# lisvulaczo/lodestar

Measured on AMD Instinct MI355X. Metric: BLS signature sets verified/sec (whole node) at 1/2/4/8 MI355X; p50 batch latency, higher is better.
Workload: dtype u32

## Files before the change

### lodestar_amd/csrc/lsg_curve.hpp

```cpp
#pragma once
#include "lsg_tower.hpp"

LSG_INL fp_t fadd(const fp_t& a, const fp_t& b) { return fp_add(a, b); }
LSG_INL fp2_t fadd(const fp2_t& a, const fp2_t& b) { return fp2_add(a, b); }
LSG_INL fp_t fsub(const fp_t& a, const fp_t& b) { return fp_sub(a, b); }
LSG_INL fp2_t fsub(const fp2_t& a, const fp2_t& b) { return fp2_sub(a, b); }
LSG_INL fp_t fmul(const fp_t& a, const fp_t& b) { return fp_mul(a, b); }
LSG_INL fp2_t fmul(const fp2_t& a, const fp2_t& b) { return fp2_mul(a, b); }
LSG_INL fp_t fsqr(const fp_t& a) { return fp_sqr(a); }
LSG_INL fp2_t fsqr(const fp2_t& a) { return fp2_sqr(a); }
LSG_INL fp_t fneg(const fp_t& a) { return fp_neg(a); }
LSG_INL fp2_t fneg(const fp2_t& a) { return fp2_neg(a); }
LSG_INL fps_t<1, 0> fsum(const fp_t& a) { return fps(a); }
LSG_INL fp2s_t<1, 0> fsum(const fp2_t& a) { return fp2s(a); }
template <int K, int P, int N>
LSG_INL fps_t<K * P, K * N> fsum_mulk(const fps_t<P, N>& a) { return fps_mulk<K>(a); }
template <int K, int P0, int N0, int P1, int N1>
LSG_INL fp2s_t<K * P0, K * N0, K * P1, K * N1> fsum_mulk(const fp2s_t<P0, N0, P1, N1>& a) { return fp2s_mulk<K>(a); }
template <int K> LSG_INL fp_t fmulk(const fp_t& a) { return fp_mulk<K>(a); }
template <int K> LSG_INL fp2_t fmulk(const fp2_t& a) { return fp2_mulk<K>(a); }
template <class F> LSG_INL F fsub2(const F& a, const F& b, const F& c) { return (fsum(a) - b - c).carry(); }
LSG_INL fp_t fmul_b3(const fp_t& a) { return fp_mul12(a); }
LSG_INL fp2_t fmul_b3(const fp2_t& a) { return fp2_mul_b3(a); }
template <int P0, int N0, int P1, int N1>
// ... 47 lines not shown

template <class F>
LSG_INL proj_t<F> proj_from_aff(const aff_t<F>& a) {
  proj_t<F> r;
  r.X = a.x;
  r.Y = a.y;
  r.Z = fone<F>();
  return r;
}

template <class F>
LSG_INL bool proj_is_inf(const proj_t<F>& a) {
  return fis_zero(a.Z);
}

template <class F>
LSG_INL proj_t<F> proj_neg(const proj_t<F>& a) {
  proj_t<F> r = a;
  r.Y = fneg(a.Y);
  return r;
}

template <class F>
LSG_INL proj_t<F> proj_add(const proj_t<F>& p, const proj_t<F>& q) {
  F t0 = fmul(p.X, q.X);
  F t1 = fmul(p.Y, q.Y);
  F t2 = fmul(p.Z, q.Z);
  F t3 = fsub2(fmul(fadd(p.X, p.Y), fadd(q.X, q.Y)), t0, t1);
  F t4 = fsub2(fmul(fadd(p.Y, p.Z), fadd(q.Y, q.Z)), t1, t2);
  F Y3 = fsub2(fmul(fadd(p.X, p.Z), fadd(q.X, q.Z)), t0, t2);
  F X3;
  t0 = fmulk<3>(t0);
  t2 = fmul_b3(t2);
  F Z3 = fadd(t1, t2);
  t1 = fsub(t1, t2);
  Y3 = fmul_b3(Y3);
  X3 = fmul(t4, Y3);
  t2 = fmul(t3, t1);
  X3 = fsub(t2, X3);
  Y3 = fmul(Y3, t0);
  t1 = fmul(t1, Z3);
  Y3 = fadd(t1, Y3);
  t0 = fmul(t0, t3);
  Z3 = fmul(Z3, t4);
  Z3 = fadd(Z3, t0);
  proj_t<F> r;
  r.X = X3;
  r.Y = Y3;
  r.Z = Z3;
  return r;
}

template <class F>
LSG_INL proj_t<F> proj_add_mixed(const proj_t<F>& p, const aff_t<F>& q) {
  F t0 = fmul(p.X, q.x);
  F t1 = fmul(p.Y, q.y);
  F t3 = fsub2(fmul(fadd(q.x, q.y), fadd(p.X, p.Y)), t0, t1);
  F t4 = fadd(fmul(q.y, p.Z), p.Y);
  F Y3 = fadd(fmul(q.x, p.Z), p.X);
  F X3;
  t0 = fmulk<3>(t0);
  F t2 = fmul_b3(p.Z);
  F Z3 = fadd(t1, t2);
  t1 = fsub(t1, t2);
  Y3 = fmul_b3(Y3);
  X3 = fmul(t4, Y3);
  t2 = fmul(t3, t1);
  X3 = fsub(t2, X3);
  Y3 = fmul(Y3, t0);
  t1 = fmul(t1, Z3);
  Y3 = fadd(t1, Y3);
  t0 = fmul(t0, t3);
  Z3 = fmul(Z3, t4);
  Z3 = fadd(Z3, t0);
  proj_t<F> r;
  r.X = X3;
  r.Y = Y3;
  r.Z = Z3;
  return r;
}

template <class F>
LSG_INL proj_t<F> proj_dbl(const proj_t<F>& p) {
  F t0 = fsqr(p.Y);
  F Z3 = fmulk<8>(t0);
  F t1 = fmul(p.Y, p.Z);
  F t2 = fmul_b3(fsqr(p.Z));
  F X3 = fmul(t2, Z3);
  F Y3 = fadd(t0, t2);
  Z3 = fmul(t1, Z3);
  t0 = fsub(t0, fmulk<3>(t2));
  Y3 = fmul(t0, Y3);
  Y3 = fadd(X3, Y3);
  t1 = fmul(p.X, p.Y);
  X3 = fmulk<2>(fmul(t0, t1));
  proj_t<F> r;
  r.X = X3;
  r.Y = Y3;
  r.Z = Z3;
  return r;
}

LSG_BIGFN g1p_t g1_add(g1p_t p, g1p_t q) { return proj_add(p, q); }
LSG_BIGFN g1p_t g1_add_mixed(g1p_t p, g1a_t q) { return proj_add_mixed(p, q); }
LSG_BIGFN g1p_t g1_dbl(g1p_t p) { return proj_dbl(p); }
LSG_BIGFN g2p_t g2_add(g2p_t p, g2p_t q) { return proj_add(p, q); }
LSG_BIGFN g2p_t g2_dbl(g2p_t p) { return proj_dbl(p); }
LSG_BIGFN g2p_t g2_add_mixed(g2p_t p, g2a_t q) { return proj_add_mixed(p, q); }

LSG_INL g1p_t gadd(const g1p_t& p, const g1p_t& q) { return g1_add(p, q); }
LSG_INL g2p_t gadd(const g2p_t& p, const g2p_t& q) { return g2_add(p, q); }
LSG_INL g1p_t gdbl(const g1p_t& p) { return g1_dbl(p); }
LSG_INL g2p_t gdbl(const g2p_t& p) { return g2_dbl(p); }
#ifdef LSG_FP2_LANES
typedef aff_t<fp2v_t> g2va_t;
typedef proj_t<fp2v_t> g2vp_t;
LSG_BIGFN g2vp_t g2v_add(g2vp_t p, g2vp_t q) { return proj_add(p, q); }
LSG_INL g2vp_t gadd(const g2vp_t& p, const g2vp_t& q) { return g2v_add(p, q); }
LSG_INL g2va_t g2v_from_pair(const g2a_t& a) { return g2va_t{fp2v_from_pair(a.x), fp2v_from_pair(a.y)}; }
LSG_INL g2vp_t g2v_from_pair(const g2p_t& p) {
  return g2vp_t{fp2v_from_pair(p.X), fp2v_from_pair(p.Y), fp2v_from_pair(p.Z)};
}
LSG_INL g2p_t g2_to_pair(const g2vp_t& p) {
  g2p_t r;
  r.X = fp2v_to_pair(p.X);
  r.Y = fp2v_to_pair(p.Y);
  r.Z = fp2v_to_pair(p.Z);
  return r;
}
#endif
LSG_INL const g2p_t& g2_to_pair(const g2p_t& p) { return p; }
template <class F> struct g2_layout;
template <> struct g2_layout<fp2_t> {
  static LSG_INL g2a_t in(const g2a_t& a) { return a; }
};
#ifdef LSG_FP2_LANES
template <> struct g2_layout<fp2v_t> {
  static LSG_INL g2va_t in(const g2a_t& a) { return g2v_from_pair(a); }
};
typedef fp2v_t chain_fp2_t;
#else
typedef fp2_t chain_fp2_t;
#endif

template <class F>
struct jac_t {
  F X, Y, Z;
};

template <class F>
LSG_INL jac_t<F> jac_from_proj(const proj_t<F>& p) {
  F zz = fsqr(p.Z);
  jac_t<F> r;
  bool inf = fis_zero(p.Z);
  r.X = fselect(inf, fone<F>(), fmul(p.X, p.Z));
  r.Y = fselect(inf, fone<F>(), fmul(p.Y, zz));
  r.Z = p.Z;
  return r;
}

template <class F>
LSG_INL proj_t<F> jac_to_proj(const jac_t<F>& p) {
  F zz = fsqr(p.Z);
  proj_t<F> r;
  bool inf = fis_zero(p.Z);
  r.X = fmul(p.X, p.Z);
  r.Y = fselect(inf, fone<F>(), p.Y);
  r.Z = fmul(zz, p.Z);
  return r;
}

template <class F>
LSG_INL jac_t<F> jac_dbl_t(const jac_t<F>& p) {
  F A = fsqr(p.X);
  F B = fsqr(p.Y);
  F C = fsqr(B);
  F D = (fsum(fsqr(fadd(p.X, B))) - A - C).template carry_mul<2>();
  F E = fmulk<3>(A);
  F Fq = fsqr(E);
  jac_t<F> r;
  r.X = (fsum(Fq) - fsum_mulk<2>(fsum(D))).carry();
  r.Y = fsub(fmul(E, fsub(D, r.X)), fmulk<8>(C));
  r.Z = fmulk<2>(fmul(p.Y, p.Z));
  return r;
}
LSG_BIGFN jac_t<fp_t> jac_dbl(jac_t<fp_t> p) { return jac_dbl_t(p); }
LSG_BIGFN jac_t<fp2_t> jac_dbl(jac_t<fp2_t> p) { return jac_dbl_t(p); }
#ifdef LSG_FP2_LANES
LSG_BIGFN jac_t<fp2v_t> jac_dbl(jac_t<fp2v_t> p) { return jac_dbl_t(p); }
#endif

template <class F>
LSG_INL jac_t<F> jac_add_proj(const jac_t<F>& acc, const proj_t<F>& q) {
  return jac_from_proj(gadd(jac_to_proj(acc), q));
}

template <class F>
LSG_INL proj_t<F> proj_mul_u64(const proj_t<F>& p, uint64_t k) {
  proj_t<F> T[16];
  T[0] = proj_inf<F>();
  T[1] = p;
  T[2] = gdbl(p);
#pragma unroll 1
  for (int d = 3; d < 16; d++) T[d] = gadd(T[d - 1], p);
  auto pick = [&](uint32_t d) { return T[d]; };
  jac_t<F> acc = jac_from_proj(pick((uint32_t)(k >> 60) & 15u));
#pragma unroll 1
  for (int w = 14; w >= 0; w--) {
    acc = jac_dbl(acc);
    acc = jac_dbl(acc);
    acc = jac_dbl(acc);
    acc = jac_dbl(acc);
    acc = jac_add_proj(acc, pick((uint32_t)(k >> (4 * w)) & 15u));
  }
  return jac_to_proj(acc);
}

template <class F>
LSG_INL proj_t<F> proj_pick_signed(const proj_t<F>& T1, const proj_t<F>& T2, const proj_t<F>& T3,
                                   const proj_t<F>& T4, int d) {
  const int a = d < 0 ? -d : d;
  proj_t<F> r = proj_inf<F>();
  auto take = [&](bool s, const proj_t<F>& t) {
    r.X = fselect(s, t.X, r.X);
    r.Y = fselect(s, t.Y, r.Y);
    r.Z = fselect(s, t.Z, r.Z);
  };
  take(a == 1, T1);
  take(a == 2, T2);
  take(a == 3, T3);
  take(a == 4, T4);
  r.Y = fselect(d < 0, fneg(r.Y), r.Y);
  return r;
}
template <class F>
LSG_INL proj_t<F> proj_mul_u64_s3(const proj_t<F>& p, uint64_t k) {
  const proj_t<F> T2 = gdbl(p);
  const proj_t<F> T3 = gadd(T2, p);
  const proj_t<F> T4 = gdbl(T2);
  uint32_t cm = 0;
#pragma unroll
  for (int i = 0; i < 21; i++) {
    const uint32_t v = (uint32_t)((k >> (3 * i)) & 7u) + ((cm >> i) & 1u);
    cm |= (v >= 4u ? 1u : 0u) << (i + 1);
  }
  auto digit = [&](int i) {
    return (int)((k >> (3 * i)) & 7u) + (int)((cm >> i) & 1u) - (i < 21 ? 8 * (int)((cm >> (i + 1)) & 1u) : 0);
  };
  jac_t<F> acc = jac_from_proj(proj_pick_signed(p, T2, T3, T4, digit(21)));
#pragma unroll 1
  for (int i = 20; i >= 0; i--) {
    acc = jac_dbl(acc);
    acc = jac_dbl(acc);
    acc = jac_dbl(acc);
    acc = jac_add_proj(acc, proj_pick_signed(p, T2, T3, T4, digit(i)));
  }
  return jac_to_proj(acc);
}

template <class F, class G>
LSG_INL proj_t<F> proj_mul_xabs_get(const G& get) {
  const uint64_t xa = ((uint64_t)LSG_X_ABS_HI << 32) | LSG_X_ABS_LO;
  jac_t<F> acc = jac_from_proj(get());
#pragma unroll 1
  for (int b = 62; b >= 0; b--) {
    acc = jac_dbl(acc);
    if ((xa >> b) & 1u) acc = jac_add_proj(acc, get());
  }
  return jac_to_proj(acc);
}
#ifdef LSG_FP2_LANES
LSG_INL jac_t<fp2v_t> jac_from_pair(const jac_t<fp2_t>& p) {
  return jac_t<fp2v_t>{fp2v_from_pair(p.X), fp2v_from_pair(p.Y), fp2v_from_pair(p.Z)};
}
LSG_INL jac_t<fp2_t> jac_to_pair(const jac_t<fp2v_t>& p) {
  jac_t<fp2_t> r;
  r.X = fp2v_to_pair(p.X);
  r.Y = fp2v_to_pair(p.Y);
  r.Z = fp2v_to_pair(p.Z);
  return r;
}
template <class G>
LSG_INL g2p_t g2_mul_xabs_get_dbl_lanes(const G& get) {
  const uint64_t xa = ((uint64_t)LSG_X_ABS_HI << 32) | LSG_X_ABS_LO;
  jac_t<fp2v_t> acc = jac_from_pair(jac_from_proj(get()));
#pragma unroll 1
  for (int b = 62; b >= 0; b--) {
    acc = jac_dbl(acc);
    if ((xa >> b) & 1u) acc = jac_from_pair(jac_add_proj(jac_to_pair(acc), get()));
  }
  return jac_to_proj(jac_to_pair(acc));
}
#endif
template <class F>
LSG_INL proj_t<F> proj_mul_xabs(const proj_t<F>& p) {
  return proj_mul_xabs_get<F>([&]() { return p; });
}

template <class F>
LSG_INL bool proj_eq(const proj_t<F>& a, const proj_t<F>& b) {
  bool ia = proj_is_inf(a), ib = proj_is_inf(b);
  if (ia || ib) return ia && ib;
  return feq(fmul(a.X, b.Z), fmul(b.X, a.Z)) && feq(fmul(a.Y, b.Z), fmul(b.Y, a.Z));
}

template <class F>
LSG_INL aff_t<F> proj_to_aff(const proj_t<F>& p) {
  F zi = finv(p.Z);
  aff_t<F> r;
  r.x = fmul(p.X, zi);
  r.y = fmul(p.Y, zi);
  return r;
}

LSG_INL g2p_t g2_psi(const g2p_t& p) {
  g2p_t r;
  r.X = fp2_mul(fp2_conj(p.X), PSI_CX);
  r.Y = fp2_mul(fp2_conj(p.Y), PSI_CY);
  r.Z = fp2_conj(p.Z);
  return r;
}
LSG_INL g2p_t g2_psi2(const g2p_t& p) {
  g2p_t r;
  r.X = fp2_mul_fp(p.X, PSI2_CX);
  r.Y = fp2_mul_fp(p.Y, PSI2_CY);
  r.Z = p.Z;
  return r;
}

template <class F = fp2_t, class G>
LSG_INL bool g2_in_group_get(const G& get) {
  if (proj_is_inf(get())) return true;
  const proj_t<F> xp = proj_neg(proj_mul_xabs_get<F>(get));
  return proj_eq(g2_psi(g2_to_pair(get())), g2_to_pair(xp));
}
LSG_BIGFN bool g2_in_group(g2p_t p) {
  return g2_in_group_get([&]() { return p; });
}

LSG_BIGFN bool g1_in_group(g1p_t p) {
  const uint32_t rw[8] = {0x73eda753u, 0x299d7d48u, 0x3339d808u, 0x09a1d805u,
                          0x53bda402u, 0xfffe5bfeu, 0xffffffffu, 0x00000001u};
  g1p_t acc = proj_inf<fp_t>();
#pragma unroll 1
  for (int w = 0; w < 8; w++) {
#pragma unroll 1
    for (int b = 31; b >= 0; b--) {
      acc = g1_dbl(acc);
      if ((rw[w] >> b) & 1u) acc = g1_add(acc, p);
    }
  }
  return proj_is_inf(acc);
}

LSG_INL bool g1_on_curve_aff(const g1a_t& a) {
  fp_t rhs = fp_add(fp_mul(fp_sqr(a.x), a.x), FP_B_G1);
  return fp_eq(fp_sqr(a.y), rhs);
}
LSG_INL bool g2_on_curve_aff(const g2a_t& a) {
  fp2_t rhs = fp2_add(fp2_mul(fp2_sqr(a.x), a.x), FP2_B_G2);
  return fp2_eq(fp2_sqr(a.y), rhs);
}

#ifndef LSG_BLST_SUCCESS
#define LSG_BLST_SUCCESS 0
#define LSG_BLST_BAD_ENCODING 1
#define LSG_BLST_POINT_NOT_ON_CURVE 2
#define LSG_BLST_POINT_NOT_IN_GROUP 3
#define LSG_BLST_AGGR_TYPE_MISMATCH 4
#define LSG_BLST_VERIFY_FAIL 5
#define LSG_BLST_PK_IS_INFINITY 6
#define LSG_BLST_BAD_SCALAR 7
#define LSG_BLST_INVALID_SIZE 10
#endif

#define LSG_UNCOMPRESS_PENDING (-1)
LSG_INL int g2_uncompress_parse(g2a_t& out, bool& inf, fp2_t& x, fp2_t& rhs, bool& want, const uint8_t* in) {
  uint8_t in0 = in[0];
  inf = false;
  if (!(in0 & 0x80)) return LSG_BLST_BAD_ENCODING;
  if (in0 & 0x40) {
    uint32_t acc = in0 & 0x3f;
    for (int i = 1; i < 96; i++) acc |= in[i];
    if (acc == 0) {
      inf = true;
      out.x = fp2_zero();
      out.y = fp2_zero();
      return LSG_BLST_SUCCESS;
    }
    return LSG_BLST_BAD_ENCODING;
  }
  fp_t x1 = fp_from_be48(in);
  x1 = fp_mask_flags(x1);
  fp_t x0 = fp_from_be48(in + 48);
  if (!fp_canon_lt_p(x1) || !fp_canon_lt_p(x0)) return LSG_BLST_BAD_ENCODING;
  x = fp2_make(fp_to_mont(x0), fp_to_mont(x1));
  rhs = fp2_add(fp2_mul(fp2_sqr(x), x), FP2_B_G2);
  want = (in0 & 0x20) != 0;
  return LSG_UNCOMPRESS_PENDING;
}
LSG_INL int g2_uncompress_finish(g2a_t& out, const fp2_t& x, fp2_t y, bool ok, bool want) {
  if (!ok) return LSG_BLST_POINT_NOT_ON_CURVE;
  if (fp2_lexi_largest(y) != want) y = fp2_neg(y);
  out.x = x;
  out.y = y;
  if (fp2_is_zero(x)) return LSG_BLST_POINT_NOT_IN_GROUP;
  return LSG_BLST_SUCCESS;
}
LSG_INL int g2_uncompress(g2a_t& out, bool& inf, const uint8_t* in) {
  fp2_t x, rhs, y;
  bool want;
  int e = g2_uncompress_parse(out, inf, x, rhs, want, in);
  if (e != LSG_UNCOMPRESS_PENDING) return e;
  bool ok = fp2_sqrt(y, rhs);
  return g2_uncompress_finish(out, x, y, ok, want);
}

// ... 100 lines not shown
```

### lodestar_amd/csrc/lsg_k_miller.hip

```cpp
#include "lsg_kcommon.hpp"

constexpr int W_LINE_LANE = (int)(sizeof(line_t) / 4);
LSG_DEVI void line_store(uint32_t* __restrict__ lines, size_t n, size_t i, int st, const line_t& L) {
  uint32_t w[W_LINE_LANE];
  __builtin_memcpy(w, &L, sizeof(line_t));
  uint32_t* p = lines + (((size_t)st * W_LINE_LANE) * n + i) * LSG_GROUP + (threadIdx.x % LSG_GROUP);
#pragma unroll
  for (int k = 0; k < W_LINE_LANE; k++) p[(size_t)k * n * LSG_GROUP] = w[k];
}
LSG_DEVI line_t line_load(const uint32_t* __restrict__ lines, size_t n, size_t i, int st) {
  uint32_t w[W_LINE_LANE];
  const uint32_t* p = lines + (((size_t)st * W_LINE_LANE) * n + i) * LSG_GROUP + (threadIdx.x % LSG_GROUP);
#pragma unroll
  for (int k = 0; k < W_LINE_LANE; k++) w[k] = p[(size_t)k * n * LSG_GROUP];
  line_t L;
  __builtin_memcpy(&L, w, sizeof(line_t));
  return L;
}

__global__ void LSG_KERNEL_ATTR k_miller_lines(int n, const uint32_t* __restrict__ H, uint32_t* __restrict__ lines) {
  LANE_ITEM(n);
  (void)lead;
  const g2a_t Q = lane_load<g2a_t>(H, item);
  miller_lines(Q, [&](int st, const line_t& L) { line_store(lines, (size_t)n, item, st, L); });
// ... 184 lines not shown
    mf_put2(lds, MF_LC(2 * pi, 1), mfc_pair<1>(V));
    mf_put2(lds, MF_LC(2 * pi, 2), V(2));
  } else {
    mf_put2(lds, MF_LC(2 * pi + 1, 0), mfc_pair<2>(V));
    mf_put2(lds, MF_LC(2 * pi + 1, 1), mfc_pair<3>(V));
  }
  __syncthreads();
}

template <class F>
LSG_DEVI void mf_mul_pair(uint32_t* lds, int w, int k) {
  {
    const F m0 = mf_get2<F>(lds, MF_LC(2 * k, 0)), m1 = mf_get2<F>(lds, MF_LC(2 * k, 1)), m2 = mf_get2<F>(lds, MF_LC(2 * k, 2));
    if (w == 0) {
      const F a0 = mf_get2<F>(lds, MF_FC(0)), a1 = mf_get2<F>(lds, MF_FC(1)), a2 = mf_get2<F>(lds, MF_FC(2));
      mf_put2(lds, MF_VC(0), fmul(a0, m0));
      mf_put2(lds, MF_VC(1), fmul(a1, m1));
      mf_put2(lds, MF_VC(2), fmul(a2, m2));
      mf_put2(lds, MF_VC(3), fmul(fadd(a0, a1), fadd(m0, m1)));
      mf_put2(lds, MF_VC(4), fmul(fadd(a1, a2), fadd(m1, m2)));
    } else if (w == 1) {
      const F m4 = mf_get2<F>(lds, MF_LC(2 * k + 1, 0)), m5 = mf_get2<F>(lds, MF_LC(2 * k + 1, 1));
      const F b0 = mf_get2<F>(lds, MF_FC(3)), b1 = mf_get2<F>(lds, MF_FC(4));
      mf_put2(lds, MF_VC(5), fmul(fadd(mf_get2<F>(lds, MF_FC(0)), mf_get2<F>(lds, MF_FC(2))), fadd(m0, m2)));
      mf_put2(lds, MF_VC(6), fmul(b0, m4));
      mf_put2(lds, MF_VC(7), fmul(b1, m5));
      mf_put2(lds, MF_VC(8), fmul(fadd(b0, b1), fadd(m4, m5)));
    } else if (w == 2) {
      const F m4 = mf_get2<F>(lds, MF_LC(2 * k + 1, 0)), m5 = mf_get2<F>(lds, MF_LC(2 * k + 1, 1));
      const F b2 = mf_get2<F>(lds, MF_FC(5));
      mf_put2(lds, MF_VC(9), fmul(b2, m4));
      mf_put2(lds, MF_VC(10), fmul(b2, m5));
      const F s0 = fadd(mf_get2<F>(lds, MF_FC(0)), mf_get2<F>(lds, MF_FC(3)));
      const F s1 = fadd(mf_get2<F>(lds, MF_FC(1)), mf_get2<F>(lds, MF_FC(4)));
      mf_put2(lds, MF_VC(11), fmul(s0, m0));
      mf_put2(lds, MF_VC(12), fmul(s1, fadd(m1, m4)));
    } else {
      const F m4 = mf_get2<F>(lds, MF_LC(2 * k + 1, 0)), m5 = mf_get2<F>(lds, MF_LC(2 * k + 1, 1));
      const F s0 = fadd(mf_get2<F>(lds, MF_FC(0)), mf_get2<F>(lds, MF_FC(3)));
      const F s1 = fadd(mf_get2<F>(lds, MF_FC(1)), mf_get2<F>(lds, MF_FC(4)));
      const F s2 = fadd(mf_get2<F>(lds, MF_FC(2)), mf_get2<F>(lds, MF_FC(5)));
      const F q1 = fadd(m1, m4), q2 = fadd(m2, m5);
      mf_put2(lds, MF_VC(13), fmul(s2, q2));
      mf_put2(lds, MF_VC(14), fmul(fadd(s0, s1), fadd(m0, q1)));
      mf_put2(lds, MF_VC(15), fmul(fadd(s1, s2), fadd(q1, q2)));
      mf_put2(lds, MF_VC(16), fmul(fadd(s0, s2), fadd(m0, q2)));
    }
  }
  __syncthreads();
  auto V = [&](int p) { return mf_get2<F>(lds, MF_VC(p)); };
  F o0, o1;
  int j0, j1 = -1;
  if (w == 0) {
    o0 = mfc_mul<0>(V);
    o1 = mfc_mul<1>(V);
    j0 = 0;
    j1 = 1;
  } else if (w == 1) {
    o0 = mfc_mul<2>(V);
    o1 = mfc_mul<3>(V);
    j0 = 2;
    j1 = 3;
  } else if (w == 2) {
    o0 = mfc_mul<4>(V);
    j0 = 4;
  } else {
    o0 = mfc_mul<5>(V);
    j0 = 5;
  }
  mf_put2(lds, MF_FC(j0), o0);
  if (j1 >= 0) mf_put2(lds, MF_FC(j1), o1);
  __syncthreads();
}

template <class F>
LSG_DEVI void mf_put_line(uint32_t* lds, int wl, bool use, const F& l00, const F& l01P, const F& l11P) {
  mf_put2(lds, MF_LC(wl, 0), fselect(use, l00, mf_layout<F>::one()));
  mf_put2(lds, MF_LC(wl, 1), fselect(use, l01P, fzero<F>()));
  mf_put2(lds, MF_LC(wl, 2), fselect(use, l11P, fzero<F>()));
}
template <class F>
LSG_DEVI void mf_dbl_line(uint32_t* lds, int wl, bool use, const uint32_t* __restrict__ P, size_t sl) {
  const int tb = MF_T + 6 * wl;
  F t0, t1, t2, v1;
  {
    const F X = mf_get2<F>(lds, tb), Y = mf_get2<F>(lds, tb + 2), Z = mf_get2<F>(lds, tb + 4);
    t0 = fsqr(Y);
    t1 = fmul(Y, Z);
    t2 = fmul_b3(fsqr(Z));
    const F XX = fsqr(X);
    v1 = fmul(X, Y);
    const g1a_t Pk = lane_load<g1a_t>(P, sl);
    mf_put_line(lds, wl, use, fsub(t2, t0), fmul_fp(fmulk<3>(XX), mf_layout<F>::fp_in(Pk.x)),
                fmul_fp((-fsum(t1)).template carry_mul<2>(), mf_layout<F>::fp_in(Pk.y)));
  }
  F Z3 = fmulk<8>(t0);
  F X3 = fmul(t2, Z3);
  F Y3 = fadd(t0, t2);
  mf_put2(lds, tb + 4, fmul(t1, Z3));
  const F s0 = (fsum(t0) - fsum_mulk<3>(fsum(t2))).carry();
  Y3 = fmul(s0, Y3);
  mf_put2(lds, tb + 2, fadd(X3, Y3));
  X3 = fmul(s0, v1);
  mf_put2(lds, tb, fmulk<2>(X3));
}
template <class F>
LSG_DEVI void mf_add_line(uint32_t* lds, int wl, bool use, const uint32_t* __restrict__ P, const uint32_t* __restrict__ H,
                          size_t sl) {
  const int tb = MF_T + 6 * wl;
  F theta, delta;
  {
    const aff_t<F> Q = g2_layout<F>::in(lane_load<g2a_t>(H, sl));
    const F Z = mf_get2<F>(lds, tb + 4);
    theta = fsub(mf_get2<F>(lds, tb + 2), fmul(Q.y, Z));
    delta = fsub(mf_get2<F>(lds, tb), fmul(Q.x, Z));
    const F l00 = fsub(fmul(delta, Q.y), fmul(theta, Q.x));
    const g1a_t Pk = lane_load<g1a_t>(P, sl);
    mf_put_line(lds, wl, use, l00, fmul_fp(theta, mf_layout<F>::fp_in(Pk.x)),
                fmul_fp(fneg(delta), mf_layout<F>::fp_in(Pk.y)));
  }
  const F C = fsqr(theta);
  const F D = fsqr(delta);
  const F E = fmul(D, delta);
  const F Fz = fmul(mf_get2<F>(lds, tb + 4), C);
  const F G = fmul(mf_get2<F>(lds, tb), D);
  const F Hs = (fsum(E) + Fz - fsum_mulk<2>(fsum(G))).carry();
  mf_put2(lds, tb, fmul(delta, Hs));
  const F Y3 = fsub(fmul(theta, fsub(G, Hs)), fmul(E, mf_get2<F>(lds, tb + 2)));
  mf_put2(lds, tb + 2, Y3);
  mf_put2(lds, tb + 4, fmul(E, mf_get2<F>(lds, tb + 4)));
}

#ifndef LSG_MF_PRIO
#define LSG_MF_PRIO 2
#endif
#ifndef LSG_MF_WAVES
#define LSG_MF_WAVES 2
#endif
#define MF_KERNEL_PARAMS                                                                                        \
  int n_items, const int32_t *__restrict__ item_first, const int32_t *__restrict__ item_cnt,                   \
      const uint32_t *__restrict__ P, const uint8_t *__restrict__ pinf, const uint8_t *__restrict__ hinf,      \
      const int32_t *__restrict__ err, const uint32_t *__restrict__ H, uint32_t *__restrict__ f_out
template <class F>
LSG_DEVI void mf_body(uint32_t* lds, MF_KERNEL_PARAMS) {
#if LSG_MF_PRIO
  __builtin_amdgcn_s_setprio(LSG_MF_PRIO);
#endif
  const int w = __builtin_amdgcn_readfirstlane((int)(threadIdx.x >> 6));
  const size_t it = (size_t)blockIdx.x * MF_ITEMS + ((threadIdx.x & 63) >> 1);
  const bool live = it < (size_t)n_items;
  const size_t itc = live ? it : 0;
  const int first = item_first[itc], cnt = item_cnt[itc];
  const int si = first + (w < cnt ? w : cnt - 1);
  const uint64_t use_mask = __ballot(live && w < cnt && err[si] == 0 && !pinf[si] && !hinf[si]);
  {
    const proj_t<F> T = proj_from_aff(g2_layout<F>::in(lane_load<g2a_t>(H, (size_t)si)));
    mf_put2(lds, MF_T + 6 * w, T.X);
    mf_put2(lds, MF_T + 6 * w + 2, T.Y);
    mf_put2(lds, MF_T + 6 * w + 4, T.Z);
  }
  auto line_phase = [&](bool add) {
    int wl = w, sl = si;
    asm volatile("" : "+s"(wl), "+v"(sl));
    const bool use = (use_mask >> __lane_id()) & 1u;
    if (add)
      mf_add_line<F>(lds, wl, use, P, H, (size_t)sl);
    else
      mf_dbl_line<F>(lds, wl, use, P, (size_t)sl);
    __syncthreads();
    mf_pair_lines<F>(lds, wl);
#pragma unroll 1
    for (int k = 0; k < 2; k++) mf_mul_pair<F>(lds, wl, k);
  };
  if (w < 2) {
    mf_put2(lds, MF_FC(3 * w), w == 0 ? fone<F>() : fzero<F>());
    mf_put2(lds, MF_FC(3 * w + 1), fzero<F>());
    mf_put2(lds, MF_FC(3 * w + 2), fzero<F>());
  }
  const uint64_t xa = ((uint64_t)LSG_X_ABS_HI << 32) | LSG_X_ABS_LO;
  line_phase(false);
  line_phase(true);
#pragma unroll 1
  for (int b = 61; b >= 0; b--) {
    int ws = w;
    asm volatile("" : "+s"(ws));
    mf_sqr<F>(lds, ws);
    line_phase(false);
// ... 77 lines not shown
```

### lodestar_amd/csrc/lsg_k_sig.hip

```cpp
#include "lsg_kcommon.hpp"

__global__ void LSG_KERNEL_ATTR k_sig_decode(int n, const uint8_t* __restrict__ sig, const uint32_t* __restrict__ sig_len,
                                             uint32_t* __restrict__ sig_aff, uint8_t* __restrict__ inf,
                                             int32_t* __restrict__ err) {
  LANE_ITEM(n);
  uint32_t len = sig_len[item];
  g2a_t p;
  p.x = fp2_zero();
  p.y = fp2_zero();
  bool is_inf = false;
  int e;
  if (len == 96)
    e = g2_uncompress(p, is_inf, sig + 192 * item);
  else if (len == 192)
    e = g2_deserialize_uncompressed(p, is_inf, sig + 192 * item);
  else
    e = LSG_BLST_INVALID_SIZE;
  lane_store(sig_aff, item, p);
  if (lead) {
    inf[item] = is_inf ? 1 : 0;
    err[item] = e;
  }
}

struct sigdec_state_t {
  fp2_t x, rhs;
  uint32_t w;
};
static_assert(lane_words<sigdec_state_t>() == lsgk::POW_SIG_STATE, "layout: decode stage state");
__global__ void LSG_KERNEL_ATTR k_sig_decode_a(int n, const uint8_t* __restrict__ sig, const uint32_t* __restrict__ sig_len,
                                               uint32_t* __restrict__ sig_aff, uint8_t* __restrict__ inf,
                                               int32_t* __restrict__ err, uint32_t* __restrict__ state,
                                               uint32_t* __restrict__ pa) {
  LANE_ITEM(n);
  uint32_t len = sig_len[item];
  g2a_t p;
  p.x = fp2_zero();
  p.y = fp2_zero();
  sigdec_state_t s;
  s.x = fp2_zero();
  s.rhs = fp2_zero();
  s.w = 0;
  fp_t pw = fp_zero();
  bool is_inf = false;
  int e;
  if (len == 96) {
    bool want = false;
    e = g2_uncompress_parse(p, is_inf, s.x, s.rhs, want, sig + 192 * item);
    if (e == LSG_UNCOMPRESS_PENDING) {
      s.w = 1u | (want ? 2u : 0u);
      pw = fp2_norm(s.rhs);
    }
  } else if (len == 192)
    e = g2_deserialize_uncompressed(p, is_inf, sig + 192 * item);
  else
    e = LSG_BLST_INVALID_SIZE;
  lane_store(state, item, s);
  lane_store(pa, item, pw);
  if (e == LSG_UNCOMPRESS_PENDING) return;
  lane_store(sig_aff, item, p);
  if (lead) {
    inf[item] = is_inf ? 1 : 0;
    err[item] = e;
  }
}
__global__ void LSG_KERNEL_ATTR k_sig_decode_b(int n, uint32_t* __restrict__ state, uint32_t* __restrict__ pa,
                                               const uint32_t* __restrict__ pb) {
  LANE_ITEM(n);
  (void)lead;
  sigdec_state_t s = lane_load<sigdec_state_t>(state, item);
  if (!(s.w & 1u)) return;
  const fp_t cand = lane_load<fp_t>(pb, item);
  if (fp_is_root_of(cand, lane_load<fp_t>(pa, item))) s.w |= 4u;
  lane_store(pa, item, fp2_sqrt_root_c(s.rhs, cand));
  lane_store(state, item, s);
}
__global__ void LSG_KERNEL_ATTR k_sig_decode_c(int n, const uint32_t* __restrict__ state, const uint32_t* __restrict__ pa,
                                               const uint32_t* __restrict__ pb, uint32_t* __restrict__ sig_aff,
                                               uint8_t* __restrict__ inf, int32_t* __restrict__ err) {
  LANE_ITEM(n);
  const sigdec_state_t s = lane_load<sigdec_state_t>(state, item);
  if (!(s.w & 1u)) return;
  fp2_t y;
  const bool root = fp2_sqrt_root_finish(y, s.rhs, lane_load<fp_t>(pa, item), lane_load<fp_t>(pb, item));
  g2a_t p;
  p.x = fp2_zero();
  p.y = fp2_zero();
  const int e = g2_uncompress_finish(p, s.x, y, (s.w & 4u) != 0 && root, (s.w & 2u) != 0);
  lane_store(sig_aff, item, p);
  if (lead) {
    inf[item] = 0;
    err[item] = e;
  }
}

template <class F>
LSG_DEVI void sig_subgroup_item(uint32_t* park, int n, const uint32_t* __restrict__ sig_aff,
                                const uint8_t* __restrict__ inf, int32_t* __restrict__ err) {
  LANE_ITEM(n);
  if (err[item] != 0 || inf[item]) return;
  lds_park(park, g2_layout<F>::in(lane_load<g2a_t>(sig_aff, item)));
  bool ok = g2_in_group_get<F>([&]() { return proj_from_aff(lds_unpark<aff_t<F>>(park)); });
  if (lead && !ok) err[item] = LSG_BLST_POINT_NOT_IN_GROUP;
}
__global__ void LSG_KERNEL_ATTR k_sig_subgroup(int n, const uint32_t* __restrict__ sig_aff,
                                               const uint8_t* __restrict__ inf, int32_t* __restrict__ err) {
  __shared__ uint32_t park[sizeof(g2a_t) / 4 * LSG_TPB];
  sig_subgroup_item<chain_fp2_t>(park, n, sig_aff, inf, err);
}
#ifdef LSG_FP2_LANES
__global__ void LSG_KERNEL_ATTR k_sig_subgroup_pair(int n, const uint32_t* __restrict__ sig_aff,
                                                    const uint8_t* __restrict__ inf, int32_t* __restrict__ err) {
  __shared__ uint32_t park[sizeof(g2a_t) / 4 * LSG_TPB];
  sig_subgroup_item<fp2_t>(park, n, sig_aff, inf, err);
}
#endif

LSG_DEVI bool sig_usable(size_t i, const uint8_t* inf, const int32_t* err, const uint8_t* pinf) {
  return err[i] == 0 && !inf[i] && !(pinf && pinf[i]);
}
__global__ void LSG_KERNEL_ATTR k_sig_proj(int n, const uint32_t* __restrict__ sig_aff, const uint8_t* __restrict__ inf,
                                           const int32_t* __restrict__ err, const uint8_t* __restrict__ pinf,
                                           uint32_t* __restrict__ out) {
  LANE_ITEM(n);
  (void)lead;
  g2p_t r = proj_inf<fp2_t>();
  if (sig_usable(item, inf, err, pinf)) r = proj_from_aff(lane_load<g2a_t>(sig_aff, item));
  lane_store(out, item, r);
}
__global__ void LSG_KERNEL_ATTR_W(1) k_sig_scale3(int n, const uint32_t* __restrict__ sig_aff, const uint8_t* __restrict__ inf,
                                                  const int32_t* __restrict__ err, const uint8_t* __restrict__ pinf,
                                                  const uint64_t* __restrict__ rnd, const uint8_t* __restrict__ mode,
                                                  uint32_t* __restrict__ out) {
  LANE_ITEM(n);
  (void)lead;
  if (mode && !mode[item]) return;
  g2p_t r = proj_inf<fp2_t>();
  if (sig_usable(item, inf, err, pinf)) {
    r = proj_from_aff(lane_load<g2a_t>(sig_aff, item));
    if (rnd[item] != 0) r = proj_mul_u64_s3(r, rnd[item]);
  }
  lane_store(out, item, r);
}

__global__ void LSG_KERNEL_ATTR k_sig_agg_seg(int n_chunks, int ips_log2, const int32_t* __restrict__ chunks,
                                              const int32_t* __restrict__ gather, const uint32_t* __restrict__ sig_aff,
                                              const uint8_t* __restrict__ inf, const int32_t* __restrict__ err,
                                              uint32_t* __restrict__ dst, uint32_t* __restrict__ tmp) {
  lsg_lane_setup();
  const size_t item = gtid() / LSG_GROUP;
  const size_t c = item >> ips_log2;
  const int ips = 1 << ips_log2, j = (int)(item & (size_t)(ips - 1));
  const bool active = c < (size_t)n_chunks;
  g2p_t acc = proj_inf<fp2_t>();
  int out = 0;
  if (active) {
    const int off = chunks[3 * c], len = chunks[3 * c + 1];
    out = chunks[3 * c + 2];
    g2a_t a;
    bool use = false;
    auto fetch = [&](int k) {
      const size_t i = (size_t)gather[off + k];
      a = lane_load<g2a_t>(sig_aff, i);
      return sig_usable(i, inf, err, nullptr);
    };
    if (j < len) use = fetch(j);
#pragma unroll 1
    for (int k = j; k < len; k += ips) {
      const g2a_t cur = a;
      const bool cur_use = use;
      if (k + ips < len) use = fetch(k + ips);
      if (cur_use) acc = proj_is_inf(acc) ? proj_from_aff(cur) : g2_add_mixed(acc, cur);
    }
  }
#pragma unroll 1
  for (int o = ips >> 1; o >= 1; o >>= 1) acc = g2_add(acc, shfl_xor_t(acc, LSG_GROUP * o));
  if (active && j == 0) {
    if (out >= 0)
      lane_store(dst, (size_t)out, acc);
    else
      lane_store(tmp, (size_t)(-out - 1), acc);
  }
}

__global__ void LSG_KERNEL_ATTR k_g2a_to_bytes(int n, const uint32_t* __restrict__ pts, const uint8_t* __restrict__ inf,
// ... 115 lines not shown
```

### lodestar_amd/csrc/lsg_pairing.hpp

```cpp
#pragma once
#include "lsg_curve.hpp"

struct line_t {
  fp2_t l00, l01, l11;
};

LSG_BIGFN line_t ml_dbl_step_raw(g2p_t& T) {
  fp2_t t0 = fp2_sqr(T.Y);
  fp2_t t1 = fp2_mul(T.Y, T.Z);
  fp2_t t2 = fp2_mul_b3(fp2_sqr(T.Z));
  fp2_t XX = fp2_sqr(T.X);
  line_t L;
  L.l00 = fp2_sub(t2, t0);
  L.l01 = fp2_mulk<3>(XX);
  L.l11 = (-fp2s(t1)).carry_mul<2>();
  fp2_t Z3 = fp2_mulk<8>(t0);
  fp2_t X3 = fp2_mul(t2, Z3);
  fp2_t Y3 = fp2_add(t0, t2);
  Z3 = fp2_mul(t1, Z3);
  fp2_t s0 = (fp2s(t0) - fp2s_mulk<3>(fp2s(t2))).carry();
  Y3 = fp2_mul(s0, Y3);
  Y3 = fp2_add(X3, Y3);
  fp2_t v1 = fp2_mul(T.X, T.Y);
  X3 = fp2_mulk<2>(fp2_mul(s0, v1));
  T.X = X3;
  T.Y = Y3;
  T.Z = Z3;
  return L;
}

LSG_BIGFN line_t ml_add_step_raw(g2p_t& T, g2a_t Q) {
  fp2_t theta = fp2_sub(T.Y, fp2_mul(Q.y, T.Z));
  fp2_t delta = fp2_sub(T.X, fp2_mul(Q.x, T.Z));
  line_t L;
  L.l00 = fp2_sub(fp2_mul(delta, Q.y), fp2_mul(theta, Q.x));
  L.l01 = theta;
  L.l11 = fp2_neg(delta);
  fp2_t C = fp2_sqr(theta);
  fp2_t D = fp2_sqr(delta);
  fp2_t E = fp2_mul(D, delta);
  fp2_t F = fp2_mul(T.Z, C);
  fp2_t G = fp2_mul(T.X, D);
  fp2_t H = (fp2s(E) + F - fp2s_mulk<2>(fp2s(G))).carry();
  fp2_t X3 = fp2_mul(delta, H);
  fp2_t Y3 = fp2_sub(fp2_mul(theta, fp2_sub(G, H)), fp2_mul(E, T.Y));
  fp2_t Z3 = fp2_mul(E, T.Z);
  T.X = X3;
  T.Y = Y3;
  T.Z = Z3;
  return L;
}

LSG_INL line_t line_eval(line_t L, const fp_t& xP, const fp_t& yP) {
  L.l01 = fp2_mul_fp(L.l01, xP);
  L.l11 = fp2_mul_fp(L.l11, yP);
  return L;
}

template <int J, class G>
LSG_INL auto mfc_sqr(const G& V) {
  if constexpr (J == 0) {
    return fp6_kar_s0(V(0), V(1), V(2), V(3)).template carry_mul<2>();
  } else if constexpr (J == 1) {
    return fp6_kar_s1(V(0), V(1), V(2), V(4)).template carry_mul<2>();
  } else if constexpr (J == 2) {
    return fp6_kar_s2(V(0), V(1), V(2), V(5)).template carry_mul<2>();
  } else if constexpr (J == 3) {
    const auto e = ((fsum(V(9)) - V(7) - V(8)) - (fsum(V(3)) - V(1) - V(2))).carry();
    const auto g = (fsum(e) - fp6_kar_s2(V(0), V(1), V(2), V(5))).carry();
    return (fsum(V(6)) - V(0) + fsum_mul_xi(g)).carry();
  } else if constexpr (J == 4) {
    const auto d = ((fsum(V(10)) - V(6) - V(7)) - (fsum(V(4)) - V(0) - V(1))).carry();
    const auto e = (fsum(d) + fsum_mul_xi(fsum(V(8)) - V(2))).carry();
    return (fsum(e) - fp6_kar_s0(V(0), V(1), V(2), V(3))).carry();
  } else {
    const auto d = ((fsum(V(11)) - V(6) - V(8)) - (fsum(V(5)) - V(0) - V(2))).carry();
    const auto t1 = fp6_kar_s1(V(0), V(1), V(2), V(4)).carry();
    return (fsum(d) + V(7) - V(1) - t1).carry();
  }
}
template <int J, class G>
LSG_INL auto mfc_pair(const G& V) {
  if constexpr (J == 0) {
    return (fsum(V(0)) + fsum_mul_xi(V(1))).carry();
  } else if constexpr (J == 1) {
    return fsub2(V(3), V(0), V(2));
  } else if constexpr (J == 2) {
    return fsub2(V(4), V(0), V(1));
  } else {
    return fsub2(V(5), V(2), V(1));
  }
}
template <int J, class G>
LSG_INL auto mfc_mul(const G& V) {
  if constexpr (J == 0) {
    const auto g = (fsum(V(4)) - V(1) - V(2) + V(8)).carry();
    const auto h = (fsum(g) - V(6) - V(7)).carry();
    return (fsum(V(0)) + fsum_mul_xi(h)).carry();
  } else if constexpr (J == 1) {
    const auto h = (fsum(V(2)) + V(7) + V(9)).carry();
    return ((fsum(V(3)) - V(0) - V(1)) + fsum_mul_xi(h)).carry();
  } else if constexpr (J == 2) {
    const auto n0 = (fsum(V(6)) + fsum_mul_xi(V(10))).carry();
    return (fsum(V(5)) - V(0) - V(2) + V(1) + n0).carry();
  } else if constexpr (J == 3) {
    const auto g = (fsum(V(15)) - V(12) - V(13) + V(1) + V(2)).carry();
    const auto h = (fsum(g) - V(4) - V(7) - V(9)).carry();
    return (fsum(V(11)) - V(0) + fsum_mul_xi(h)).carry();
  } else if constexpr (J == 4) {
    const auto a = ((fsum(V(14)) - V(11) - V(12)) - (fsum(V(3)) - V(0) - V(1))).carry();
    const auto b = fsub2(V(13), V(2), V(10));
    return (fsum(a) - V(6) + fsum_mul_xi(b)).carry();
  } else {
    const auto g = (fsum(V(11)) + V(13) + V(5) - V(16) - V(12) - V(0)).carry();
    return (fsum(V(2)) + V(6) + V(7) - V(1) - V(8) - g).carry();
  }
}

LSG_INL line_t ml_dbl_step(g2p_t& T, fp_t xP, fp_t yP) { return line_eval(ml_dbl_step_raw(T), xP, yP); }

LSG_INL line_t ml_add_step(g2p_t& T, g2a_t Q, fp_t xP, fp_t yP) {
  return line_eval(ml_add_step_raw(T, Q), xP, yP);
}

LSG_BIGFN fp12_t miller_loop(g1a_t P, g2a_t Q) {
  const uint64_t xa = ((uint64_t)LSG_X_ABS_HI << 32) | LSG_X_ABS_LO;
  g2p_t T = proj_from_aff(Q);
  line_t L = ml_dbl_step(T, P.x, P.y);
  fp12_t f;
  f.c0 = fp6_make(L.l00, L.l01, fp2_zero());
  f.c1 = fp6_make(fp2_zero(), L.l11, fp2_zero());
  L = ml_add_step(T, Q, P.x, P.y);
  f = fp12_mul_line(f, L.l00, L.l01, L.l11);
  for (int b = 61; b >= 0; b--) {
    f = fp12_sqr(f);
    L = ml_dbl_step(T, P.x, P.y);
    f = fp12_mul_line(f, L.l00, L.l01, L.l11);
    if ((xa >> b) & 1u) {
      L = ml_add_step(T, Q, P.x, P.y);
// ... 125 lines not shown
```

Measured before the change: 3.928 million.

## Use squaring-based projective doubling, mixed adds, and homogeneous G1 scalar mul

Rewrites projective doubling and the Miller-loop doubling line so that several multiplications become squarings, using (Y+Z)^2-B-C style identities and a squared form for Y3. The G1 3-bit signed scalar multiplication now runs in homogeneous projective coordinates instead of converting to Jacobian, and the subgroup check passes affine points so that mixed addition is used. The aim is fewer full field multiplications in the hot curve and pairing paths. The cost is extra additions and carries, and a risk of correctness bugs in the new formulas (for example the sign of the l11 coefficient and the line slot layout).

```diff
diff --git a/lodestar_amd/csrc/lsg_curve.hpp b/lodestar_amd/csrc/lsg_curve.hpp
--- a/lodestar_amd/csrc/lsg_curve.hpp
+++ b/lodestar_amd/csrc/lsg_curve.hpp
@@ -153,22 +153,16 @@
 
 template <class F>
 LSG_INL proj_t<F> proj_dbl(const proj_t<F>& p) {
-  F t0 = fsqr(p.Y);
-  F Z3 = fmulk<8>(t0);
-  F t1 = fmul(p.Y, p.Z);
-  F t2 = fmul_b3(fsqr(p.Z));
-  F X3 = fmul(t2, Z3);
-  F Y3 = fadd(t0, t2);
-  Z3 = fmul(t1, Z3);
-  t0 = fsub(t0, fmulk<3>(t2));
-  Y3 = fmul(t0, Y3);
-  Y3 = fadd(X3, Y3);
-  t1 = fmul(p.X, p.Y);
-  X3 = fmulk<2>(fmul(t0, t1));
+  const F B = fsqr(p.Y);
+  const F C = fsqr(p.Z);
+  const F yz2 = fsub2(fsqr(fadd(p.Y, p.Z)), B, C);
+  const F E = fmul_b3(C);
   proj_t<F> r;
-  r.X = X3;
-  r.Y = Y3;
-  r.Z = Z3;
+  r.Z = fmul(fmulk<4>(B), yz2);
+  const F s0 = (fsum(B) - fsum_mulk<3>(fsum(E))).carry();
+  const F s1 = (fsum_mulk<2>(fsum(B)) - s0).carry();
+  r.Y = fsub(fsqr(s1), fmulk<12>(fsqr(E)));
+  r.X = fmulk<2>(fmul(s0, fmul(p.X, p.Y)));
   return r;
 }
 
@@ -183,11 +177,15 @@
 LSG_INL g2p_t gadd(const g2p_t& p, const g2p_t& q) { return g2_add(p, q); }
 LSG_INL g1p_t gdbl(const g1p_t& p) { return g1_dbl(p); }
 LSG_INL g2p_t gdbl(const g2p_t& p) { return g2_dbl(p); }
+LSG_INL g1p_t gadd(const g1p_t& p, const g1a_t& q) { return g1_add_mixed(p, q); }
+LSG_INL g2p_t gadd(const g2p_t& p, const g2a_t& q) { return g2_add_mixed(p, q); }
 #ifdef LSG_FP2_LANES
 typedef aff_t<fp2v_t> g2va_t;
 typedef proj_t<fp2v_t> g2vp_t;
 LSG_BIGFN g2vp_t g2v_add(g2vp_t p, g2vp_t q) { return proj_add(p, q); }
+LSG_BIGFN g2vp_t g2v_add_mixed(g2vp_t p, g2va_t q) { return proj_add_mixed(p, q); }
 LSG_INL g2vp_t gadd(const g2vp_t& p, const g2vp_t& q) { return g2v_add(p, q); }
+LSG_INL g2vp_t gadd(const g2vp_t& p, const g2va_t& q) { return g2v_add_mixed(p, q); }
 LSG_INL g2va_t g2v_from_pair(const g2a_t& a) { return g2va_t{fp2v_from_pair(a.x), fp2v_from_pair(a.y)}; }
 LSG_INL g2vp_t g2v_from_pair(const g2p_t& p) {
   return g2vp_t{fp2v_from_pair(p.X), fp2v_from_pair(p.Y), fp2v_from_pair(p.Z)};
@@ -261,10 +259,12 @@
 LSG_BIGFN jac_t<fp2v_t> jac_dbl(jac_t<fp2v_t> p) { return jac_dbl_t(p); }
 #endif
 
-template <class F>
-LSG_INL jac_t<F> jac_add_proj(const jac_t<F>& acc, const proj_t<F>& q) {
+template <class F, class Q>
+LSG_INL jac_t<F> jac_add_proj(const jac_t<F>& acc, const Q& q) {
   return jac_from_proj(gadd(jac_to_proj(acc), q));
 }
+template <class F> LSG_INL const proj_t<F>& proj_of(const proj_t<F>& p) { return p; }
+template <class F> LSG_INL proj_t<F> proj_of(const aff_t<F>& a) { return proj_from_aff(a); }
 
 template <class F>
 LSG_INL proj_t<F> proj_mul_u64(const proj_t<F>& p, uint64_t k) {
@@ -304,6 +304,8 @@
   r.Y = fselect(d < 0, fneg(r.Y), r.Y);
   return r;
 }
+template <class F> struct s3_homogeneous { static constexpr bool value = false; };
+template <> struct s3_homogeneous<fp_t> { static constexpr bool value = true; };
 template <class F>
 LSG_INL proj_t<F> proj_mul_u64_s3(const proj_t<F>& p, uint64_t k) {
   const proj_t<F> T2 = gdbl(p);
@@ -318,21 +320,33 @@
   auto digit = [&](int i) {
     return (int)((k >> (3 * i)) & 7u) + (int)((cm >> i) & 1u) - (i < 21 ? 8 * (int)((cm >> (i + 1)) & 1u) : 0);
   };
-  jac_t<F> acc = jac_from_proj(proj_pick_signed(p, T2, T3, T4, digit(21)));
-#pragma unroll 1
-  for (int i = 20; i >= 0; i--) {
-    acc = jac_dbl(acc);
-    acc = jac_dbl(acc);
-    acc = jac_dbl(acc);
-    acc = jac_add_proj(acc, proj_pick_signed(p, T2, T3, T4, digit(i)));
-  }
-  return jac_to_proj(acc);
+  if constexpr (s3_homogeneous<F>::value) {
+    proj_t<F> acc = proj_pick_signed(p, T2, T3, T4, digit(21));
+#pragma unroll 1
+    for (int i = 20; i >= 0; i--) {
+      acc = gdbl(acc);
+      acc = gdbl(acc);
+      acc = gdbl(acc);
+      acc = gadd(acc, proj_pick_signed(p, T2, T3, T4, digit(i)));
+    }
+    return acc;
+  } else {
+    jac_t<F> acc = jac_from_proj(proj_pick_signed(p, T2, T3, T4, digit(21)));
+#pragma unroll 1
+    for (int i = 20; i >= 0; i--) {
+      acc = jac_dbl(acc);
+      acc = jac_dbl(acc);
+      acc = jac_dbl(acc);
+      acc = jac_add_proj(acc, proj_pick_signed(p, T2, T3, T4, digit(i)));
+    }
+    return jac_to_proj(acc);
+  }
 }
 
 template <class F, class G>
 LSG_INL proj_t<F> proj_mul_xabs_get(const G& get) {
   const uint64_t xa = ((uint64_t)LSG_X_ABS_HI << 32) | LSG_X_ABS_LO;
-  jac_t<F> acc = jac_from_proj(get());
+  jac_t<F> acc = jac_from_proj(proj_of<F>(get()));
 #pragma unroll 1
   for (int b = 62; b >= 0; b--) {
     acc = jac_dbl(acc);
@@ -401,9 +415,9 @@
 
 template <class F = fp2_t, class G>
 LSG_INL bool g2_in_group_get(const G& get) {
-  if (proj_is_inf(get())) return true;
+  if (proj_is_inf(proj_of<F>(get()))) return true;
   const proj_t<F> xp = proj_neg(proj_mul_xabs_get<F>(get));
-  return proj_eq(g2_psi(g2_to_pair(get())), g2_to_pair(xp));
+  return proj_eq(g2_psi(g2_to_pair(proj_of<F>(get()))), g2_to_pair(xp));
 }
 LSG_BIGFN bool g2_in_group(g2p_t p) {
   return g2_in_group_get([&]() { return p; });
diff --git a/lodestar_amd/csrc/lsg_k_miller.hip b/lodestar_amd/csrc/lsg_k_miller.hip
--- a/lodestar_amd/csrc/lsg_k_miller.hip
+++ b/lodestar_amd/csrc/lsg_k_miller.hip
@@ -290,27 +290,15 @@
 template <class F>
 LSG_DEVI void mf_dbl_line(uint32_t* lds, int wl, bool use, const uint32_t* __restrict__ P, size_t sl) {
   const int tb = MF_T + 6 * wl;
-  F t0, t1, t2, v1;
-  {
-    const F X = mf_get2<F>(lds, tb), Y = mf_get2<F>(lds, tb + 2), Z = mf_get2<F>(lds, tb + 4);
-    t0 = fsqr(Y);
-    t1 = fmul(Y, Z);
-    t2 = fmul_b3(fsqr(Z));
-    const F XX = fsqr(X);
-    v1 = fmul(X, Y);
-    const g1a_t Pk = lane_load<g1a_t>(P, sl);
-    mf_put_line(lds, wl, use, fsub(t2, t0), fmul_fp(fmulk<3>(XX), mf_layout<F>::fp_in(Pk.x)),
-                fmul_fp((-fsum(t1)).template carry_mul<2>(), mf_layout<F>::fp_in(Pk.y)));
-  }
-  F Z3 = fmulk<8>(t0);
-  F X3 = fmul(t2, Z3);
-  F Y3 = fadd(t0, t2);
-  mf_put2(lds, tb + 4, fmul(t1, Z3));
-  const F s0 = (fsum(t0) - fsum_mulk<3>(fsum(t2))).carry();
-  Y3 = fmul(s0, Y3);
-  mf_put2(lds, tb + 2, fadd(X3, Y3));
-  X3 = fmul(s0, v1);
-  mf_put2(lds, tb, fmulk<2>(X3));
+  ml_dbl_line_sq<F>(
+      [&]() { return proj_t<F>{mf_get2<F>(lds, tb), mf_get2<F>(lds, tb + 2), mf_get2<F>(lds, tb + 4)}; },
+      [&]() { return lane_load<g1a_t>(P, sl); }, [](const fp_t& a) { return mf_layout<F>::fp_in(a); },
+      [&](int slot, const F& v) {
+        if (slot < 3)
+          mf_put2(lds, MF_LC(wl, slot), fselect(use, v, slot == 0 ? mf_layout<F>::one() : fzero<F>()));
+        else
+          mf_put2(lds, tb + 2 * (slot - 3), v);
+      });
 }
 template <class F>
 LSG_DEVI void mf_add_line(uint32_t* lds, int wl, bool use, const uint32_t* __restrict__ P, const uint32_t* __restrict__ H,
diff --git a/lodestar_amd/csrc/lsg_k_sig.hip b/lodestar_amd/csrc/lsg_k_sig.hip
--- a/lodestar_amd/csrc/lsg_k_sig.hip
+++ b/lodestar_amd/csrc/lsg_k_sig.hip
@@ -100,7 +100,7 @@
   LANE_ITEM(n);
   if (err[item] != 0 || inf[item]) return;
   lds_park(park, g2_layout<F>::in(lane_load<g2a_t>(sig_aff, item)));
-  bool ok = g2_in_group_get<F>([&]() { return proj_from_aff(lds_unpark<aff_t<F>>(park)); });
+  bool ok = g2_in_group_get<F>([&]() { return lds_unpark<aff_t<F>>(park); });
   if (lead && !ok) err[item] = LSG_BLST_POINT_NOT_IN_GROUP;
 }
 __global__ void LSG_KERNEL_ATTR k_sig_subgroup(int n, const uint32_t* __restrict__ sig_aff,
diff --git a/lodestar_amd/csrc/lsg_pairing.hpp b/lodestar_amd/csrc/lsg_pairing.hpp
--- a/lodestar_amd/csrc/lsg_pairing.hpp
+++ b/lodestar_amd/csrc/lsg_pairing.hpp
@@ -55,6 +55,29 @@
   L.l01 = fp2_mul_fp(L.l01, xP);
   L.l11 = fp2_mul_fp(L.l11, yP);
   return L;
+}
+
+template <class F, class GetT, class GetP, class FpIn, class Put>
+LSG_INL void ml_dbl_line_sq(const GetT& getT, const GetP& getP, const FpIn& fp_in, const Put& put) {
+  F B, E, yz2, xy2;
+  {
+    const proj_t<F> T = getT();
+    B = fsqr(T.Y);
+    const F C = fsqr(T.Z);
+    yz2 = fsub2(fsqr(fadd(T.Y, T.Z)), B, C);
+    E = fmul_b3(C);
+    const F J = fsqr(T.X);
+    xy2 = fsub2(fsqr(fadd(T.X, T.Y)), J, B);
+    const g1a_t Pk = getP();
+    put(0, fsub(E, B));
+    put(1, fmul_fp(fmulk<3>(J), fp_in(Pk.x)));
+    put(2, fmul_fp(yz2, fp_in(fp_neg(Pk.y))));
+  }
+  put(5, fmul(fmulk<4>(B), yz2));
+  const F s0 = (fsum(B) - fsum_mulk<3>(fsum(E))).carry();
+  put(3, fmul(s0, xy2));
+  const F s1 = (fsum_mulk<2>(fsum(B)) - s0).carry();
+  put(4, fsub(fsqr(s1), fmulk<12>(fsqr(E))));
 }
 
 template <int J, class G>
```

After: 4.020 million (median of 6 runs). +2.3%, better.
